# xingyizhou/CenterNet

Hardware: AMD Instinct MI355X
Metric: images/sec whole-node, 512x512 ctdet (higher is better)
Workload: dtype f32s; 1 GPU; ctdet resdcn_18 512x512, batch 32 per GPU (BASELINE configs[1]), network + fused sigmoid/peak-NMS/top-K decode, K=100; global_batch=32, parallelism=image-sharded x1

## Files before the change

centernet_amd/csrc/cn_heads_at.hip:

```cpp
#include "cn_common.h"
#include "cn_internal.h"

namespace {

constexpr int HA_NT = 256;
constexpr int HA_CELLS = 16;
constexpr int HA_CC = 64;
constexpr int HA_ROW = 9 * HA_CC;
constexpr int HA_MAXN = 512;
constexpr int HA_PF = 4;

struct HeadsAtArgs {
    const char *feat;
    const float *scores;
    const int32_t *inds, *clses;
    const cn_f32x4 *w1;
    const float *b1;
    const float *w2;
    const float *b2;
    float *dets;
    float *vals;
    float mul;
    int H, W, Cin, pitch, K, hidden, n_heads, N;
};

template <bool F32S, int CT, int NS>
__global__ __launch_bounds__(HA_NT) void decode_heads_at_cells_kernel(const HeadsAtArgs a)
{
    constexpr int CG = HA_CELLS / CT;
    constexpr int TPC = HA_NT / CG;
    static_assert(TPC % 64 == 0, "the lanes of a wave read one cell's patch");
    __shared__ __attribute__((aligned(16))) float lds[HA_CELLS * HA_ROW];
    __shared__ int s_ind[HA_CELLS];
    __shared__ float s_out[HA_CELLS * 4];

    const int tid = threadIdx.x;
    const int b = blockIdx.y;
    const int k0 = blockIdx.x * HA_CELLS;
    const int ncell = min(HA_CELLS, a.K - k0);
    const int HW = a.H * a.W;
    const int N = a.N;

    if (tid < HA_CELLS) {
        int ind = -1;
        if (tid < ncell) {
            ind = a.inds[(size_t)b * a.K + k0 + tid];
            if ((uint32_t)ind >= (uint32_t)HW) ind = -1;
        }
        s_ind[tid] = ind;
    }

    const int nl = tid % TPC, cg = tid / TPC;
    float acc[NS][CT];
#pragma unroll
    for (int s = 0; s < NS; ++s)
#pragma unroll
        for (int i = 0; i < CT; ++i) acc[s][i] = 0.f;

    size_t kq_base = 0;
    for (int c0 = 0; c0 < a.Cin; c0 += HA_CC) {
        const int cc = min(HA_CC, a.Cin - c0);
        const int cq = cc >> 2;
        __syncthreads();
        for (int i = tid; i < HA_CELLS * 9 * cq; i += HA_NT) {
            const int q = i % cq, r = i / cq;
            const int tap = r % 9, cell = r / 9;
            const int ind = s_ind[cell];
            cn_f32x4 v = {0.f, 0.f, 0.f, 0.f};
            if (ind >= 0) {
                const int y = ind / a.W + tap / 3 - 1, x = ind % a.W + tap % 3 - 1;
                if ((unsigned)y < (unsigned)a.H && (unsigned)x < (unsigned)a.W) {
                    const size_t pix = ((size_t)b * a.H + y) * a.W + x;
                    if (F32S) {
                        v = cn_load4_f32s(a.feat, pix, a.pitch, c0 + 4 * q);
                        v *= a.mul;
                    } else {
                        v = *reinterpret_cast<const cn_f32x4 *>(a.feat + (pix * (size_t)a.pitch + c0 + 4 * q) * 4);
                    }
                }
            }
            *reinterpret_cast<cn_f32x4 *>(&lds[cell * HA_ROW + tap * cc + 4 * q]) = v;
        }
        __syncthreads();

        const int nkq = 9 * cq;
        const cn_f32x4 *wq = a.w1 + kq_base * N;
        cn_f32x4 wn[HA_PF][NS];
#pragma unroll
        for (int p = 0; p < HA_PF; ++p)
#pragma unroll
            for (int s = 0; s < NS; ++s) {
                const int n = nl + s * TPC;
                wn[p][s] = n < N ? wq[(size_t)p * N + n] : cn_f32x4{0.f, 0.f, 0.f, 0.f};
            }
        for (int kq = 0; kq < nkq; kq += HA_PF) {
            cn_f32x4 wv[HA_PF][NS];
#pragma unroll
            for (int p = 0; p < HA_PF; ++p)
#pragma unroll
                for (int s = 0; s < NS; ++s) wv[p][s] = wn[p][s];
            if (kq + HA_PF < nkq) {
#pragma unroll
                for (int p = 0; p < HA_PF; ++p)
#pragma unroll
                    for (int s = 0; s < NS; ++s) {
                        const int n = nl + s * TPC;
                        if (n < N) wn[p][s] = wq[(size_t)(kq + HA_PF + p) * N + n];
                    }
            }
#pragma unroll
            for (int p = 0; p < HA_PF; ++p)
#pragma unroll
                for (int i = 0; i < CT; ++i) {
                    const cn_f32x4 pv = *reinterpret_cast<const cn_f32x4 *>(&lds[(i * CG + cg) * HA_ROW + 4 * (kq + p)]);
#pragma unroll
                    for (int s = 0; s < NS; ++s) {
                        float t = acc[s][i];
                        t = __builtin_fmaf(wv[p][s][0], pv[0], t);
                        t = __builtin_fmaf(wv[p][s][1], pv[1], t);
                        t = __builtin_fmaf(wv[p][s][2], pv[2], t);
                        t = __builtin_fmaf(wv[p][s][3], pv[3], t);
                        acc[s][i] = t;
                    }
                }
        }
        kq_base += (size_t)nkq;
    }

    __syncthreads();
#pragma unroll
    for (int s = 0; s < NS; ++s) {
        const int n = nl + s * TPC;
        if (n < N) {
            const float bias = a.b1[n];
#pragma unroll
            for (int i = 0; i < CT; ++i)
                lds[(i * CG + cg) * HA_ROW + n] = __builtin_fmaxf(acc[s][i] + bias, 0.f);
        }
    }
    __syncthreads();

    {
        const int o = tid >> 2, sub = tid & 3;
        const int cell = o >> 2, head = (o >> 1) & 1, j = o & 1;
        float sum = 0.f;
        if (head < a.n_heads) {
            const float *w = a.w2 + ((size_t)head * 2 + j) * a.hidden;
            const float *h = &lds[cell * HA_ROW + head * a.hidden];
            for (int c = sub; c < a.hidden; c += 4) sum = __builtin_fmaf(w[c], h[c], sum);
        }
        sum += __shfl_xor(sum, 1);
        sum += __shfl_xor(sum, 2);
        if (sub == 0) {
            if (head < a.n_heads && a.b2) sum += a.b2[head * 2 + j];
            s_out[o] = sum;
        }
    }
    __syncthreads();

    if (tid < ncell) {
        const size_t row = (size_t)b * a.K + k0 + tid;
        const int ind = s_ind[tid];
        float *d = a.dets + row * 6;
        const float score = a.scores[row];
        const float cls = (float)a.clses[row];
        if (ind < 0) {
            const float nan = __builtin_nanf("");
            d[0] = nan; d[1] = nan; d[2] = nan; d[3] = nan; d[4] = score; d[5] = cls;
            if (a.vals)
                for (int v = 0; v < 2 * a.n_heads; ++v) a.vals[row * (2 * a.n_heads) + v] = nan;
            return;
        }
        const int yi = ind / a.W, xi = ind - yi * a.W;
        float xs = (float)xi, ys = (float)yi;
        if (a.n_heads > 1) {
            xs = xs + s_out[tid * 4 + 2];
            ys = ys + s_out[tid * 4 + 3];
        } else {
            xs = xs + 0.5f;
            ys = ys + 0.5f;
        }
        const float w = s_out[tid * 4 + 0];
        const float h = s_out[tid * 4 + 1];
        d[0] = xs - w / 2;
        d[1] = ys - h / 2;
        d[2] = xs + w / 2;
        d[3] = ys + h / 2;
        d[4] = score;
        d[5] = cls;
        if (a.vals)
            for (int v = 0; v < 2 * a.n_heads; ++v) a.vals[row * (2 * a.n_heads) + v] = s_out[tid * 4 + v];
    }
}

__global__ void decode_pack_cell_w1_kernel(const float *__restrict__ w, float *__restrict__ out, int N, int Cin,
                                           size_t total)
{
    const size_t i = (size_t)blockIdx.x * blockDim.x + threadIdx.x;
    if (i >= total) return;
    const int e = (int)(i & 3);
    const int n = (int)((i >> 2) % N);
    const int k = (int)((i >> 2) / N) * 4 + e;
    const int chunk = k / (9 * HA_CC);
    const int c0 = chunk * HA_CC;
    const int cc = min(HA_CC, Cin - c0);
    const int r = k - chunk * 9 * HA_CC;
    const int tap = r / cc, ci = c0 + r % cc;
    out[i] = w[((size_t)n * Cin + ci) * 9 + tap];
}

}

extern "C" int cn_pack_cell_heads_w1(const float *w, float *out, int N, int Cin, void *stream)
{
    if (!w || !out) return CN_ERR_NULL;
    if (N <= 0 || Cin <= 0) return CN_ERR_SHAPE;
    if (N > HA_MAXN || (N & 63) || (Cin & 31)) return CN_ERR_UNSUPPORTED;
    if (!cn_aligned16(out)) return CN_ERR_ALIGN;
    const size_t total = (size_t)N * Cin * 9;
    hipLaunchKernelGGL(decode_pack_cell_w1_kernel, dim3((unsigned)((total + 255) / 256)), dim3(256), 0,
                       (hipStream_t)stream, w, out, N, Cin, total);
    CN_CHECK_LAUNCH();
    return CN_OK;
}

extern "C" int cn_ctdet_heads_at_cells_f32(const void *feat, int B, int H, int W, int Cin, int pitch, int dtype,
                                           float feat_mul, const float *scores, const int32_t *inds,
                                           const int32_t *clses, int K, const float *w1_packed,
                                           const float *bias1, int hidden, int n_heads, const float *w2,
                                           const float *bias2, float *dets, float *head_vals, void *stream)
{
    if (!feat || !scores || !inds || !clses || !w1_packed || !bias1 || !w2 || !dets) return CN_ERR_NULL;
    if (B <= 0 || H <= 0 || W <= 0 || Cin <= 0 || K <= 0 || pitch < Cin) return CN_ERR_SHAPE;
    if (dtype != CN_DTYPE_F32S && dtype != CN_DTYPE_F32) return CN_ERR_UNSUPPORTED;
    if (n_heads < 1 || n_heads > 2 || hidden < 64 || hidden > 256 || (hidden & 63)) return CN_ERR_UNSUPPORTED;
    if ((Cin & 31) || (pitch & 3) || (dtype == CN_DTYPE_F32S && (pitch & 31))) return CN_ERR_UNSUPPORTED;
    if ((long)H * W >= (1L << 31) || B > 65535) return CN_ERR_UNSUPPORTED;
    if (!cn_aligned16(feat) || !cn_aligned16(w1_packed)) return CN_ERR_ALIGN;
    HeadsAtArgs a;
    a.feat = (const char *)feat; a.scores = scores; a.inds = inds; a.clses = clses;
    a.w1 = (const cn_f32x4 *)w1_packed; a.b1 = bias1; a.w2 = w2; a.b2 = bias2;
    a.dets = dets; a.vals = head_vals; a.mul = dtype == CN_DTYPE_F32S ? feat_mul : 1.f;
    a.H = H; a.W = W; a.Cin = Cin; a.pitch = pitch; a.K = K; a.hidden = hidden; a.n_heads = n_heads;
    a.N = hidden * n_heads;
    const dim3 grid((unsigned)cn_cdiv(K, HA_CELLS), (unsigned)B), block(HA_NT);
    hipStream_t st = (hipStream_t)stream;
    const bool s = dtype == CN_DTYPE_F32S;
#define HA_LAUNCH(CT, NS)                                                                               \
    do {                                                                                                \
        if (s) hipLaunchKernelGGL((decode_heads_at_cells_kernel<true, CT, NS>), grid, block, 0, st, a); \
        else hipLaunchKernelGGL((decode_heads_at_cells_kernel<false, CT, NS>), grid, block, 0, st, a);  \
    } while (0)
    if (a.N <= 64) HA_LAUNCH(4, 1);
    else if (a.N <= 128) HA_LAUNCH(8, 1);
    else if (a.N <= 256) HA_LAUNCH(16, 1);
    else HA_LAUNCH(16, 2);
#undef HA_LAUNCH
    CN_CHECK_LAUNCH();
    return CN_OK;
}
```

Measured before the change: 12570 img/s.

## Restructure decode heads kernel with paired-cell packed FMA and double-buffered prefetch

Halves cells per block to double the grid, interleaves pairs of cells in LDS so that packed two-wide FMAs can process two cells per weight value, and double-buffers the weight prefetch (ping-pong wa/wb) with LDS patch prefetch one step ahead. The feature gather now issues all global loads before any LDS stores to raise memory-level parallelism. It also clamps indices instead of branching. The costs are higher register pressure and more per-block fixed overhead, in a small decode-stage kernel that is likely a minor part of whole-network time.

```diff
diff --git a/centernet_amd/csrc/cn_heads_at.hip b/centernet_amd/csrc/cn_heads_at.hip
--- a/centernet_amd/csrc/cn_heads_at.hip
+++ b/centernet_amd/csrc/cn_heads_at.hip
@@ -3,12 +3,14 @@
 
 namespace {
 
+typedef float cn_f32x2 __attribute__((ext_vector_type(2)));
+
 constexpr int HA_NT = 256;
-constexpr int HA_CELLS = 16;
+constexpr int HA_CELLS = 8;
+constexpr int HA_PF = 12;
 constexpr int HA_CC = 64;
 constexpr int HA_ROW = 9 * HA_CC;
 constexpr int HA_MAXN = 512;
-constexpr int HA_PF = 4;
 
 struct HeadsAtArgs {
     const char *feat;
@@ -27,21 +29,28 @@
 template <bool F32S, int CT, int NS>
 __global__ __launch_bounds__(HA_NT) void decode_heads_at_cells_kernel(const HeadsAtArgs a)
 {
-    constexpr int CG = HA_CELLS / CT;
+    constexpr int CELLS = HA_CELLS;
+    constexpr int PF = HA_PF / NS;
+    constexpr int CG = CELLS / CT;
+    constexpr int CP = CT / 2;
+    static_assert(CT % 2 == 0, "cells go in pairs");
     constexpr int TPC = HA_NT / CG;
+    constexpr int SJ = (CELLS * 9 * (HA_CC / 4) + HA_NT - 1) / HA_NT;
     static_assert(TPC % 64 == 0, "the lanes of a wave read one cell's patch");
-    __shared__ __attribute__((aligned(16))) float lds[HA_CELLS * HA_ROW];
-    __shared__ int s_ind[HA_CELLS];
-    __shared__ float s_out[HA_CELLS * 4];
+    static_assert(72 % (2 * PF) == 0, "a chunk has 72 or 144 float4 groups");
+    static_assert(CELLS * 16 <= HA_NT, "four lanes per 1x1 output");
+    __shared__ __attribute__((aligned(16))) float lds[CELLS * HA_ROW];
+    __shared__ int s_ind[CELLS];
+    __shared__ float s_out[CELLS * 4];
 
     const int tid = threadIdx.x;
     const int b = blockIdx.y;
-    const int k0 = blockIdx.x * HA_CELLS;
-    const int ncell = min(HA_CELLS, a.K - k0);
+    const int k0 = blockIdx.x * CELLS;
+    const int ncell = min(CELLS, a.K - k0);
     const int HW = a.H * a.W;
     const int N = a.N;
 
-    if (tid < HA_CELLS) {
+    if (tid < CELLS) {
         int ind = -1;
         if (tid < ncell) {
             ind = a.inds[(size_t)b * a.K + k0 + tid];
@@ -51,78 +60,109 @@
     }
 
     const int nl = tid % TPC, cg = tid / TPC;
-    float acc[NS][CT];
+    cn_f32x2 acc[NS][CP];
 #pragma unroll
     for (int s = 0; s < NS; ++s)
 #pragma unroll
-        for (int i = 0; i < CT; ++i) acc[s][i] = 0.f;
+        for (int i = 0; i < CP; ++i) acc[s][i] = cn_f32x2{0.f, 0.f};
 
     size_t kq_base = 0;
     for (int c0 = 0; c0 < a.Cin; c0 += HA_CC) {
         const int cc = min(HA_CC, a.Cin - c0);
         const int cq = cc >> 2;
-        __syncthreads();
-        for (int i = tid; i < HA_CELLS * 9 * cq; i += HA_NT) {
-            const int q = i % cq, r = i / cq;
-            const int tap = r % 9, cell = r / 9;
-            const int ind = s_ind[cell];
-            cn_f32x4 v = {0.f, 0.f, 0.f, 0.f};
-            if (ind >= 0) {
-                const int y = ind / a.W + tap / 3 - 1, x = ind % a.W + tap % 3 - 1;
-                if ((unsigned)y < (unsigned)a.H && (unsigned)x < (unsigned)a.W) {
-                    const size_t pix = ((size_t)b * a.H + y) * a.W + x;
-                    if (F32S) {
-                        v = cn_load4_f32s(a.feat, pix, a.pitch, c0 + 4 * q);
-                        v *= a.mul;
-                    } else {
-                        v = *reinterpret_cast<const cn_f32x4 *>(a.feat + (pix * (size_t)a.pitch + c0 + 4 * q) * 4);
-                    }
-                }
-            }
-            *reinterpret_cast<cn_f32x4 *>(&lds[cell * HA_ROW + tap * cc + 4 * q]) = v;
-        }
-        __syncthreads();
-
         const int nkq = 9 * cq;
         const cn_f32x4 *wq = a.w1 + kq_base * N;
-        cn_f32x4 wn[HA_PF][NS];
-#pragma unroll
-        for (int p = 0; p < HA_PF; ++p)
+        cn_f32x4 wa[PF][NS], wb[PF][NS];
+#pragma unroll
+        for (int p = 0; p < PF; ++p)
 #pragma unroll
             for (int s = 0; s < NS; ++s) {
-                const int n = nl + s * TPC;
-                wn[p][s] = n < N ? wq[(size_t)p * N + n] : cn_f32x4{0.f, 0.f, 0.f, 0.f};
-            }
-        for (int kq = 0; kq < nkq; kq += HA_PF) {
-            cn_f32x4 wv[HA_PF][NS];
-#pragma unroll
-            for (int p = 0; p < HA_PF; ++p)
-#pragma unroll
-                for (int s = 0; s < NS; ++s) wv[p][s] = wn[p][s];
-            if (kq + HA_PF < nkq) {
-#pragma unroll
-                for (int p = 0; p < HA_PF; ++p)
+                const int n = min(nl + s * TPC, N - 1);
+                wa[p][s] = wq[(size_t)p * N + n];
+            }
+        __syncthreads();
+        {
+            const int total = CELLS * 9 * cq;
+            cn_f32x4 sv[SJ];
+            bool ok[SJ];
+#pragma unroll
+            for (int j = 0; j < SJ; ++j) {
+                const int i = min(tid + j * HA_NT, total - 1);
+                const int q = i % cq, r = i / cq;
+                const int tap = r % 9, cell = r / 9;
+                const int ind = s_ind[cell];
+                const int y = ind / a.W + tap / 3 - 1, x = ind % a.W + tap % 3 - 1;
+                ok[j] = ind >= 0 && (unsigned)y < (unsigned)a.H && (unsigned)x < (unsigned)a.W;
+                const size_t pix = (size_t)b * HW + (ok[j] ? y * a.W + x : 0);
+                if (F32S) {
+                    sv[j] = cn_load4_f32s(a.feat, pix, a.pitch, c0 + 4 * q);
+                } else {
+                    sv[j] = *reinterpret_cast<const cn_f32x4 *>(a.feat + (pix * (size_t)a.pitch + c0 + 4 * q) * 4);
+                }
+            }
+#pragma unroll
+            for (int j = 0; j < SJ; ++j) {
+                const int i = tid + j * HA_NT;
+                if (i < total) {
+                    const int q = i % cq, r = i / cq;
+                    const int tap = r % 9, cell = r / 9;
+                    cn_f32x4 v = sv[j];
+                    if (F32S) v *= a.mul;
+                    if (!ok[j]) v = cn_f32x4{0.f, 0.f, 0.f, 0.f};
+                    float *d = &lds[((cell >> 1) * HA_ROW + tap * cc + 4 * q) * 2 + (cell & 1)];
+                    d[0] = v[0]; d[2] = v[1]; d[4] = v[2]; d[6] = v[3];
+                }
+            }
+        }
+        __syncthreads();
+
+        cn_f32x4 pv[CP][2];
+#pragma unroll
+        for (int i = 0; i < CP; ++i) {
+            pv[i][0] = *reinterpret_cast<const cn_f32x4 *>(&lds[(i * CG + cg) * (2 * HA_ROW)]);
+            pv[i][1] = *reinterpret_cast<const cn_f32x4 *>(&lds[(i * CG + cg) * (2 * HA_ROW) + 4]);
+        }
+        auto half = [&](cn_f32x4 (&wc)[PF][NS], cn_f32x4 (&wnx)[PF][NS], const int k) {
+#pragma unroll
+            for (int p = 0; p < PF; ++p) {
+                const int gn = min(k + p + 1, nkq - 1);
+                cn_f32x4 pn[CP][2];
+#pragma unroll
+                for (int i = 0; i < CP; ++i) {
+                    pn[i][0] = *reinterpret_cast<const cn_f32x4 *>(&lds[(i * CG + cg) * (2 * HA_ROW) + 8 * gn]);
+                    pn[i][1] = *reinterpret_cast<const cn_f32x4 *>(&lds[(i * CG + cg) * (2 * HA_ROW) + 8 * gn + 4]);
+                }
+#pragma unroll
+                for (int i = 0; i < CP; ++i) {
 #pragma unroll
                     for (int s = 0; s < NS; ++s) {
-                        const int n = nl + s * TPC;
-                        if (n < N) wn[p][s] = wq[(size_t)(kq + HA_PF + p) * N + n];
-                    }
-            }
-#pragma unroll
-            for (int p = 0; p < HA_PF; ++p)
-#pragma unroll
-                for (int i = 0; i < CT; ++i) {
-                    const cn_f32x4 pv = *reinterpret_cast<const cn_f32x4 *>(&lds[(i * CG + cg) * HA_ROW + 4 * (kq + p)]);
-#pragma unroll
-                    for (int s = 0; s < NS; ++s) {
-                        float t = acc[s][i];
-                        t = __builtin_fmaf(wv[p][s][0], pv[0], t);
-                        t = __builtin_fmaf(wv[p][s][1], pv[1], t);
-                        t = __builtin_fmaf(wv[p][s][2], pv[2], t);
-                        t = __builtin_fmaf(wv[p][s][3], pv[3], t);
+                        const cn_f32x4 w = wc[p][s];
+                        cn_f32x2 t = acc[s][i];
+                        t = __builtin_elementwise_fma(cn_f32x2{w[0], w[0]}, cn_f32x2{pv[i][0][0], pv[i][0][1]}, t);
+                        t = __builtin_elementwise_fma(cn_f32x2{w[1], w[1]}, cn_f32x2{pv[i][0][2], pv[i][0][3]}, t);
+                        t = __builtin_elementwise_fma(cn_f32x2{w[2], w[2]}, cn_f32x2{pv[i][1][0], pv[i][1][1]}, t);
+                        t = __builtin_elementwise_fma(cn_f32x2{w[3], w[3]}, cn_f32x2{pv[i][1][2], pv[i][1][3]}, t);
                         acc[s][i] = t;
                     }
                 }
+                const int gw = min(k + PF + p, nkq - 1);
+                asm volatile("" ::: "memory");
+#pragma unroll
+                for (int s = 0; s < NS; ++s) {
+                    const int n = min(nl + s * TPC, N - 1);
+                    wnx[p][s] = wq[(size_t)gw * N + n];
+                }
+                asm volatile("" ::: "memory");
+#pragma unroll
+                for (int i = 0; i < CP; ++i) {
+                    pv[i][0] = pn[i][0];
+                    pv[i][1] = pn[i][1];
+                }
+            }
+        };
+        for (int kq = 0; kq < nkq; kq += 2 * PF) {
+            half(wa, wb, kq);
+            half(wb, wa, kq + PF);
         }
         kq_base += (size_t)nkq;
     }
@@ -134,8 +174,10 @@
         if (n < N) {
             const float bias = a.b1[n];
 #pragma unroll
-            for (int i = 0; i < CT; ++i)
-                lds[(i * CG + cg) * HA_ROW + n] = __builtin_fmaxf(acc[s][i] + bias, 0.f);
+            for (int i = 0; i < CP; ++i) {
+                lds[(2 * (i * CG + cg)) * HA_ROW + n] = __builtin_fmaxf(acc[s][i][0] + bias, 0.f);
+                lds[(2 * (i * CG + cg) + 1) * HA_ROW + n] = __builtin_fmaxf(acc[s][i][1] + bias, 0.f);
+            }
         }
     }
     __syncthreads();
@@ -143,16 +185,17 @@
     {
         const int o = tid >> 2, sub = tid & 3;
         const int cell = o >> 2, head = (o >> 1) & 1, j = o & 1;
+        const bool live = o < CELLS * 4 && head < a.n_heads;
         float sum = 0.f;
-        if (head < a.n_heads) {
+        if (live) {
             const float *w = a.w2 + ((size_t)head * 2 + j) * a.hidden;
             const float *h = &lds[cell * HA_ROW + head * a.hidden];
             for (int c = sub; c < a.hidden; c += 4) sum = __builtin_fmaf(w[c], h[c], sum);
         }
         sum += __shfl_xor(sum, 1);
         sum += __shfl_xor(sum, 2);
-        if (sub == 0) {
-            if (head < a.n_heads && a.b2) sum += a.b2[head * 2 + j];
+        if (sub == 0 && o < CELLS * 4) {
+            if (live && a.b2) sum += a.b2[head * 2 + j];
             s_out[o] = sum;
         }
     }
@@ -251,10 +294,10 @@
         if (s) hipLaunchKernelGGL((decode_heads_at_cells_kernel<true, CT, NS>), grid, block, 0, st, a); \
         else hipLaunchKernelGGL((decode_heads_at_cells_kernel<false, CT, NS>), grid, block, 0, st, a);  \
     } while (0)
-    if (a.N <= 64) HA_LAUNCH(4, 1);
-    else if (a.N <= 128) HA_LAUNCH(8, 1);
-    else if (a.N <= 256) HA_LAUNCH(16, 1);
-    else HA_LAUNCH(16, 2);
+    if (a.N <= 64) HA_LAUNCH(2, 1);
+    else if (a.N <= 128) HA_LAUNCH(4, 1);
+    else if (a.N <= 256) HA_LAUNCH(8, 1);
+    else HA_LAUNCH(8, 2);
 #undef HA_LAUNCH
     CN_CHECK_LAUNCH();
     return CN_OK;
```

Result: no change. 12520 img/s (median of 3 runs) (-0.4%).
